# Asunatan/LM-Net

Hardware: AMD Instinct MI355X
Metric: train images/sec at 352x352, 1/2/4/8 MI355X; Dice vs ref (higher is better)
Workload: dtype f32; 1 GPU; LM-Net fp32 training step (fwd + CE/Dice loss + bwd + AdamW), batch 8/GPU, 352x352 synthetic disc masks (BASELINE configs[1]); global_batch=8, parallelism=dp1, launch=lmn_plan_run (recorded C-side schedule, one crossing per pass)

## Files before the change

### lm_net_amd/csrc/conv_wgrad.hip

```cpp
#include "conv_common.h"

namespace {

struct WgradParams {
  LmnLay lay_src[3], lay_dy;
  int32_t rpw;
  uint32_t rp_magic;
  lmn_wgrad_args_t a;
  int ntile_src[3];
  int ntile_off[3];
  int cbase[3];
  int NNTT, NMTT;
  int Cin;
  int nsets_n;
  int steps_per_img;
  int total_steps;
  float inv_keep_src[3];
  float inv_keep_dy;
  float* partial;
  int TH, TW, XH, XW, CSx, CSy, tiles_x, tiles_y, total_tiles;
  uint32_t mXW, mTW;
  int dbg;
};

__device__ __forceinline__ float* wgrad_dst(const WgradParams& P, int co, int sidx, int ch, int taps) {
  float* own = P.a.dW_src[sidx];
  return own ? own + ((int64_t)co * P.a.src[sidx].C + ch) * taps
             : P.a.dW + ((int64_t)co * P.Cin + P.cbase[sidx] + ch) * taps;
}

template <int TAPS, int NMT, int NNT, int PM = 0>
__global__ __launch_bounds__(256, 2) void wgrad_lds_kernel(const WgradParams P) {
  constexpr bool BF = PM >= 1;
  typedef typename ActT<PM>::type TA;
  const lmn_wgrad_args_t& A = P.a;
  const uint32_t soff = A.seed_ctr ? *A.seed_ctr : 0u;
  extern __shared__ __attribute__((aligned(16))) float smem[];
  const int XP = P.XH * P.XW;
  float* XS = smem;
  float* YS = smem + NNT * XP * P.CSx;
  const int tid = threadIdx.x, lane = tid & 63;
  const int wv = __builtin_amdgcn_readfirstlane(tid >> 6);
  const int q = lane >> 4, n = lane & 15;
  const int mset = blockIdx.y / P.nsets_n, nset = blockIdx.y - mset * P.nsets_n;
  const int mt0 = mset * NMT, nt0 = nset * NNT;
  const int pad = A.ksize >> 1;
  const int NP = P.TH * P.TW;

  const TA* tptr[NNT];
  const float* tscale[NNT];
  int tC[NNT], tcs[NNT], tflags[NNT], tch0[NNT];
  uint32_t tseed[NNT];
  float tp_[NNT], tik[NNT];
#pragma unroll
  for (int t = 0; t < NNT; ++t) {
    const int nt = nt0 + t;
    int sidx = 0;
    while (sidx + 1 < A.nsrc && nt >= P.ntile_off[sidx + 1]) ++sidx;
    tptr[t] = (const TA*)A.src[sidx].ptr;
    tscale[t] = A.src[sidx].scale;
    tC[t] = nt < P.NNTT ? A.src[sidx].C : 0;
    tcs[t] = A.src[sidx].cstride;
    tflags[t] = A.src[sidx].flags;
    tseed[t] = A.src[sidx].drop_seed + soff;
    tp_[t] = A.src[sidx].drop_p;
    tik[t] = P.inv_keep_src[sidx];
    tch0[t] = (nt - P.ntile_off[sidx]) * 16;
  }

  f32x4 acc[TAPS][NMT][NNT];
  float bsum[NMT];
#pragma unroll
  for (int tp = 0; tp < TAPS; ++tp)
#pragma unroll
    for (int m = 0; m < NMT; ++m)
#pragma unroll
      for (int t = 0; t < NNT; ++t) acc[tp][m][t] = f32x4{0.f, 0.f, 0.f, 0.f};
#pragma unroll
  for (int m = 0; m < NMT; ++m) bsum[m] = 0.f;

  const int t_begin = (int)(((int64_t)blockIdx.x * P.total_tiles) / gridDim.x);
  const int t_end = (int)(((int64_t)(blockIdx.x + 1) * P.total_tiles) / gridDim.x);
  for (int tile = t_begin; tile < t_end; ++tile) {
    const int b = tile / (P.tiles_x * P.tiles_y), tt = tile - b * P.tiles_x * P.tiles_y;
    const int oy0 = (tt / P.tiles_x) * P.TH, ox0 = (tt % P.tiles_x) * P.TW;
    const int iy0 = oy0 * A.stride - pad, ix0 = ox0 * A.stride - pad;
    __syncthreads();
    constexpr int UX = (TAPS == 9 && NMT * NNT == 4) ? 3 : 4, UY = 2;
    const int NXI = P.XH * P.XW * 4, NYI = NP * 4;
    for (int rd = 0; rd * (UX * 256) < NXI || rd * (UY * 256) < NYI; ++rd) {
      f32x4 vx[UX][NNT], vy[UY][NMT];
      int gpx[UX], gpy[UY];
#pragma unroll
      for (int u = 0; u < UX; ++u) {
        const int i = rd * (UX * 256) + u * 256 + tid;
        const int j = i & 3, pix = i >> 2;
        bool inb;
        int gp;
        if constexpr (TAPS == 1) {
          inb = i < NXI && ox0 + pix < A.Wout;
          gp = inb ? b * A.Wout + ox0 + pix : 0;
        } else {
          const int r = (int)__umulhi((uint32_t)pix, P.mXW), c = pix - r * P.XW;
          const int iy = iy0 + r, ix = ix0 + c;
          inb = i < NXI && (unsigned)iy < (unsigned)A.Hin && (unsigned)ix < (unsigned)A.Win;
// ... 754 lines not shown
      for (int h = 0; h < U / 4; ++h) {
        uint2 af[NMT], bf[NNT];
#pragma unroll
        for (int m = 0; m < NMT; ++m) {
          bsum[m] += (av[4 * h][m] + av[4 * h + 1][m]) + (av[4 * h + 2][m] + av[4 * h + 3][m]);
          af[m] = uint2{pk_bf16(av[4 * h][m], av[4 * h + 1][m]), pk_bf16(av[4 * h + 2][m], av[4 * h + 3][m])};
        }
#pragma unroll
        for (int t = 0; t < NNT; ++t) bf[t] = uint2{pk_bf16(bv[4 * h][t], bv[4 * h + 1][t]), pk_bf16(bv[4 * h + 2][t], bv[4 * h + 3][t])};
#pragma unroll
        for (int t = 0; t < NNT; ++t)
#pragma unroll
          for (int m = 0; m < NMT; ++m) acc[m][t] = mfma_bf16(af[m], bf[t], acc[m][t]);
      }
    } else {
#pragma unroll
    for (int u = 0; u < U; ++u) {
#pragma unroll
      for (int m = 0; m < NMT; ++m) bsum[m] += av[u][m];
#pragma unroll
      for (int t = 0; t < NNT; ++t)
#pragma unroll
        for (int m = 0; m < NMT; ++m) acc[m][t] = __builtin_amdgcn_mfma_f32_16x16x4f32(av[u][m], bv[u][t], acc[m][t], 0, 0, 0);
    }
    }
  }

  constexpr int NT = NMT * NNT;
  __shared__ float s_acc[NT * 256 + NMT * 16];
  for (int w = 0; w < 4; ++w) {
    if (wvb == w) {
#pragma unroll
      for (int m = 0; m < NMT; ++m)
#pragma unroll
        for (int t = 0; t < NNT; ++t)
#pragma unroll
          for (int r = 0; r < 4; ++r) {
            float* d = &s_acc[((m * NNT + t) * 4 + r) * 64 + lane];
            *d = (w == 0) ? acc[m][t][r] : *d + acc[m][t][r];
          }
#pragma unroll
      for (int m = 0; m < NMT; ++m) {
        float v = bsum[m];
        v += __shfl_xor(v, 16, 64);
        v += __shfl_xor(v, 32, 64);
        if (q == 0) {
          float* d = &s_acc[NT * 256 + m * 16 + n];
          *d = (w == 0) ? v : *d + v;
        }
      }
    }
    __syncthreads();
  }
  const int tid = threadIdx.x;
  if (P.partial) {
    float* dst = P.partial + ((int64_t)blockIdx.y * gridDim.x + blockIdx.x) * (NT * 256 + NMT * 16);
    for (int i = tid; i < NT * 256 + NMT * 16; i += 256) dst[i] = s_acc[i];
    return;
  }
  for (int i = tid; i < NT * 256; i += 256) {
    const int ln = i & 63, r = (i >> 6) & 3, tl = i >> 8;
    const int t = tl % NNT, m = tl / NNT;
    const int qq = ln >> 4, nn = ln & 15;
    const int co = (mt0 + m) * 16 + qq * 4 + r;
    const int nt = nt0 + t;
    if ((mt0 + m) >= P.NMTT || co >= A.Cout || nt >= P.NNTT) continue;
    int sidx = 0;
    while (sidx + 1 < A.nsrc && nt >= P.ntile_off[sidx + 1]) ++sidx;
    const int ch = (nt - P.ntile_off[sidx]) * 16 + nn;
    if (ch >= A.src[sidx].C) continue;
    atomicAdd(wgrad_dst(P, co, sidx, ch, 1), s_acc[i]);
  }
  if (A.db && nset == 0) {
    for (int i = tid; i < NMT * 16; i += 256) {
      const int co = mt0 * 16 + i;
      if (co < A.Cout && (mt0 + i / 16) < P.NMTT) {
        atomicAdd(A.db + co, s_acc[NT * 256 + i]);
        if (A.db2) atomicAdd(A.db2 + co, s_acc[NT * 256 + i]);
      }
    }
  }
}

template <int NMT, int NNT, int PM>
__global__ __launch_bounds__(256) void wgrad_1x1w_kernel(const WgradParams P) {
  constexpr int PMB = PM & 3;
  constexpr bool RP = (PM & 4) != 0;
  constexpr bool BF = PMB >= 1;
  typedef typename ActT<PMB>::type TA;
  constexpr int NTT = NMT + NNT;
  const lmn_wgrad_args_t& A = P.a;
  const uint32_t soff = A.seed_ctr ? *A.seed_ctr : 0u;
  extern __shared__ __attribute__((aligned(16))) float smem[];
  const int lane = threadIdx.x & 63;
  const int q = lane >> 4, n = lane & 15;
  const int wvb = __builtin_amdgcn_readfirstlane(threadIdx.x >> 6);
  float* WS = smem + wvb * (NTT * 256);
  const int wave = blockIdx.x * 4 + wvb, nwaves = gridDim.x * 4;
  const int mset = blockIdx.y / P.nsets_n, nset = blockIdx.y - mset * P.nsets_n;
  const int mt0 = mset * NMT, nt0 = nset * NNT;
  const int HW = A.Hout * A.Wout;
  const int NPX = A.B * HW;
  const int lp = lane >> 2, lq = lane & 3;
  constexpr int LNOFF = (4 * NTT * 256 > NMT * NNT * 256 + NMT * 16) ? 4 * NTT * 256 : NMT * NNT * 256 + NMT * 16;
  float* s_gb = smem + LNOFF;
  const bool ln = (A.src[0].flags & LMN_SRC_LN) != 0;
  if (ln) {
    for (int i = threadIdx.x; i < NNT * 16; i += 256) {
      const int t = i >> 4, c = i & 15, ch = (nt0 + t) * 16 + c;
      const bool cok = (nt0 + t) < P.NNTT && ch < A.src[0].C;
      s_gb[t * 32 + c] = cok ? A.src[0].ln_gamma[ch] : 0.f;
      s_gb[t * 32 + 16 + c] = cok ? A.src[0].ln_beta[ch] : 0.f;
    }
    __syncthreads();
  }
  float2 lnmr = float2{0.f, 1.f};

  const TA* sptr[NNT];
  const float* sscale[NNT];
  int sC[NNT], scs[NNT], sflags[NNT], sch4[NNT];
  uint32_t scho[NNT], srf[NNT];
  uint32_t sseed[NNT];
  float sp[NNT], sik[NNT];
#pragma unroll
  for (int t = 0; t < NNT; ++t) {
    const int nt = nt0 + t;
    int s = 0;
    while (s + 1 < A.nsrc && nt >= P.ntile_off[s + 1]) ++s;
    const int ch = (nt - P.ntile_off[s]) * 16 + lq * 4;
    sptr[t] = (const TA*)A.src[s].ptr;
    sscale[t] = A.src[s].scale;
    sC[t] = A.src[s].C;
    scs[t] = RP ? P.lay_src[s].cs : A.src[s].cstride;
    srf[t] = RP ? (uint32_t)P.lay_src[s].rf : 0u;
    sflags[t] = A.src[s].flags;
    sseed[t] = A.src[s].drop_seed + soff;
    sp[t] = A.src[s].drop_p;
    sik[t] = P.inv_keep_src[s];
    sch4[t] = (nt < P.NNTT && ch < A.src[s].C) ? ch : -1;
    scho[t] = (uint32_t)((sch4[t] >= 0 ? sch4[t] : 0) >> 2) * (uint32_t)P.lay_src[s].qs;
  }
  int mco4[NMT];
#pragma unroll
  for (int m = 0; m < NMT; ++m) mco4[m] = ((mt0 + m) < P.NMTT && (mt0 + m) * 16 + lq * 4 < A.Cout) ? (mt0 + m) * 16 + lq * 4 : -1;
  uint32_t mcho[NMT];
#pragma unroll
  for (int m = 0; m < NMT; ++m) mcho[m] = (uint32_t)((mco4[m] >= 0 ? mco4[m] : 0) >> 2) * (uint32_t)P.lay_dy.qs;

  f32x4 acc[NMT][NNT];
  float bsum[NMT];
#pragma unroll
  for (int m = 0; m < NMT; ++m) {
    bsum[m] = 0.f;
#pragma unroll
    for (int t = 0; t < NNT; ++t) acc[m][t] = f32x4{0.f, 0.f, 0.f, 0.f};
  }

  const int total_chunks = (NPX + 15) >> 4;
  const int cb = (int)(((int64_t)wave * total_chunks) / nwaves), ce = (int)(((int64_t)(wave + 1) * total_chunks) / nwaves);
  f32x4 stg[NTT];
  auto chunk_load = [&](int c) {
    const int px = c * 16 + lp;
    const int ps = px < NPX ? px : 0;
    if (ln) lnmr = *reinterpret_cast<const float2*>(A.src[0].ln_stats + 2 * (int64_t)ps);
    if constexpr (RP) {
      const uint32_t rowp = lmn_div_row((uint32_t)ps, (uint32_t)P.rpw, P.rp_magic);
#pragma unroll
      for (int m = 0; m < NMT; ++m) stg[m] = ld4((const TA*)A.dy + ((uint32_t)(ps * P.lay_dy.cs) + mcho[m] + rowp * (uint32_t)P.lay_dy.rf));
#pragma unroll
      for (int t = 0; t < NNT; ++t) stg[NMT + t] = ld4(sptr[t] + ((uint32_t)(ps * scs[t]) + scho[t] + rowp * srf[t]));
    } else {
#pragma unroll
      for (int m = 0; m < NMT; ++m) stg[m] = ld4((const TA*)A.dy + (uint32_t)(ps * A.dy_cstride + (mco4[m] >= 0 ? mco4[m] : 0)));
#pragma unroll
      for (int t = 0; t < NNT; ++t) stg[NMT + t] = ld4(sptr[t] + (uint32_t)(ps * scs[t] + (sch4[t] >= 0 ? sch4[t] : 0)));
    }
  };
  auto chunk_put = [&](int c) {
    const int px = c * 16 + lp;
    const bool ok = px < NPX;
    const int ps = ok ? px : 0;
#pragma unroll
    for (int m = 0; m < NMT; ++m) {
      f32x4 v = stg[m];
      if (A.dy_flags & LMN_SRC_DROP) {
#pragma unroll
        for (int k = 0; k < 4; ++k) v[k] *= lmn_drop_scale(A.dy_seed + soff, (uint32_t)(ps * A.Cout + (mco4[m] >= 0 ? mco4[m] : 0) + k), A.dy_p, P.inv_keep_dy);
      }
      if (!(ok && mco4[m] >= 0)) v = f32x4{0.f, 0.f, 0.f, 0.f};
      *reinterpret_cast<f32x4*>(&WS[m * 256 + lp * 16 + lq * 4]) = v;
    }
#pragma unroll
    for (int t = 0; t < NNT; ++t) {
      f32x4 v = stg[NMT + t];
      const int chs = sch4[t] >= 0 ? sch4[t] : 0;
      if (ln) v = (v - lnmr.x) * lnmr.y * (*reinterpret_cast<const f32x4*>(&s_gb[t * 32 + lq * 4])) + (*reinterpret_cast<const f32x4*>(&s_gb[t * 32 + 16 + lq * 4]));
      if (sflags[t] & LMN_SRC_GELU) {
#pragma unroll
        for (int k = 0; k < 4; ++k) v[k] = lmn_gelu(v[k]);
      }
      if (sflags[t] & LMN_SRC_DROP) {
#pragma unroll
        for (int k = 0; k < 4; ++k) v[k] *= lmn_drop_scale(sseed[t], (uint32_t)(ps * sC[t] + chs + k), sp[t], sik[t]);
      }
      if (sscale[t]) v *= ld4(sscale[t] + (ps / HW) * sC[t] + chs);
      if (!(ok && sch4[t] >= 0)) v = f32x4{0.f, 0.f, 0.f, 0.f};
      *reinterpret_cast<f32x4*>(&WS[(NMT + t) * 256 + lp * 16 + lq * 4]) = v;
    }
  };
  if (cb < ce) chunk_load(cb);
  for (int c = cb; c < ce; ++c) {
    chunk_put(c);
    if (c + 1 < ce) chunk_load(c + 1);
    if constexpr (BF) {
      uint2 af[NMT], bf_[NNT];
#pragma unroll
      for (int m = 0; m < NMT; ++m) {
        const float a0 = WS[m * 256 + (4 * q) * 16 + n], a1 = WS[m * 256 + (4 * q + 1) * 16 + n];
        const float a2 = WS[m * 256 + (4 * q + 2) * 16 + n], a3 = WS[m * 256 + (4 * q + 3) * 16 + n];
        bsum[m] += (a0 + a1) + (a2 + a3);
        af[m] = uint2{pk_bf16(a0, a1), pk_bf16(a2, a3)};
      }
#pragma unroll
      for (int t = 0; t < NNT; ++t) {
        const float* b = &WS[(NMT + t) * 256 + (4 * q) * 16 + n];
        bf_[t] = uint2{pk_bf16(b[0], b[16]), pk_bf16(b[32], b[48])};
      }
#pragma unroll
      for (int t = 0; t < NNT; ++t)
#pragma unroll
        for (int m = 0; m < NMT; ++m) acc[m][t] = mfma_bf16(af[m], bf_[t], acc[m][t]);
    } else {
#pragma unroll
      for (int k = 0; k < 4; ++k) {
        float av[NMT], bv[NNT];
#pragma unroll
        for (int m = 0; m < NMT; ++m) av[m] = WS[m * 256 + (4 * k + q) * 16 + n];
#pragma unroll
        for (int t = 0; t < NNT; ++t) bv[t] = WS[(NMT + t) * 256 + (4 * k + q) * 16 + n];
#pragma unroll
        for (int m = 0; m < NMT; ++m) bsum[m] += av[m];
#pragma unroll
        for (int t = 0; t < NNT; ++t)
#pragma unroll
          for (int m = 0; m < NMT; ++m) acc[m][t] = __builtin_amdgcn_mfma_f32_16x16x4f32(av[m], bv[t], acc[m][t], 0, 0, 0);
      }
    }
  }

  constexpr int NT = NMT * NNT;
  __syncthreads();
  float* s_acc = smem;
  for (int w = 0; w < 4; ++w) {
    if (wvb == w) {
#pragma unroll
      for (int m = 0; m < NMT; ++m)
#pragma unroll
        for (int t = 0; t < NNT; ++t)
#pragma unroll
          for (int r = 0; r < 4; ++r) {
            float* d = &s_acc[((m * NNT + t) * 4 + r) * 64 + lane];
            *d = (w == 0) ? acc[m][t][r] : *d + acc[m][t][r];
          }
#pragma unroll
      for (int m = 0; m < NMT; ++m) {
        float v = bsum[m];
        v += __shfl_xor(v, 16, 64);
        v += __shfl_xor(v, 32, 64);
        if (q == 0) {
          float* d = &s_acc[NT * 256 + m * 16 + n];
          *d = (w == 0) ? v : *d + v;
        }
      }
    }
    __syncthreads();
  }
  const int tid = threadIdx.x;
  if (P.partial) {
    float* dst = P.partial + ((int64_t)blockIdx.y * gridDim.x + blockIdx.x) * (NT * 256 + NMT * 16);
    for (int i = tid; i < NT * 256 + NMT * 16; i += 256) dst[i] = s_acc[i];
    return;
  }
  for (int i = tid; i < NT * 256; i += 256) {
    const int ln = i & 63, r = (i >> 6) & 3, tl = i >> 8;
    const int t = tl % NNT, m = tl / NNT;
    const int qq = ln >> 4, nn = ln & 15;
    const int co = (mt0 + m) * 16 + qq * 4 + r;
    const int nt = nt0 + t;
    if ((mt0 + m) >= P.NMTT || co >= A.Cout || nt >= P.NNTT) continue;
    int sidx = 0;
    while (sidx + 1 < A.nsrc && nt >= P.ntile_off[sidx + 1]) ++sidx;
    const int ch = (nt - P.ntile_off[sidx]) * 16 + nn;
    if (ch >= A.src[sidx].C) continue;
    atomicAdd(wgrad_dst(P, co, sidx, ch, 1), s_acc[i]);
  }
  if (A.db && nset == 0) {
    for (int i = tid; i < NMT * 16; i += 256) {
      const int co = mt0 * 16 + i;
      if (co < A.Cout && (mt0 + i / 16) < P.NMTT) {
        atomicAdd(A.db + co, s_acc[NT * 256 + i]);
        if (A.db2) atomicAdd(A.db2 + co, s_acc[NT * 256 + i]);
      }
    }
  }
}

template <int TAPS, int NMT, int NNT>
__global__ __launch_bounds__(1024) void wgrad_reduce_kernel(const WgradParams P, int nblk, int ksl) {
  const lmn_wgrad_args_t& A = P.a;
  constexpr int NT = TAPS * NMT * NNT, PER = NT * 256 + NMT * 16;
  __shared__ __attribute__((aligned(16))) float red[4096];
  const int mset = blockIdx.y / P.nsets_n, nset = blockIdx.y - mset * P.nsets_n;
  const int mt0 = mset * NMT, nt0 = nset * NNT;
  const float* src = P.partial + (int64_t)blockIdx.y * nblk * PER;
  const int epq = 1024 / ksl, epb = epq * 4;
  const int q = threadIdx.x & (epq - 1), ks = threadIdx.x / epq;
  const int i4 = (blockIdx.x * epq + q) * 4;
  f32x4 s4 = f32x4{0.f, 0.f, 0.f, 0.f};
  if (i4 < PER) {
    const float* sp = src + i4;
#pragma unroll 4
    for (int k = ks; k < nblk; k += ksl) s4 += *reinterpret_cast<const f32x4*>(sp + (int64_t)k * PER);
  }
  *reinterpret_cast<f32x4*>(&red[threadIdx.x * 4]) = s4;
  __syncthreads();
  for (int e = threadIdx.x; e < epb; e += 1024) {
  const int i = blockIdx.x * epb + e;
  if (i >= PER) return;
  float sum = 0.f;
  for (int k = 0; k < ksl; ++k) sum += red[k * epb + e];
  if (i < NT * 256) {
// ... 162 lines not shown
};

static int wgrad_setup(const lmn_wgrad_args_t& A, WgradParams& P, WgGeom& G) {
  LMN_REQUIRE(A.ksize == 1 || A.ksize == 3, "conv_wgrad: ksize %d", A.ksize);
  LMN_REQUIRE(A.stride == 1 || A.stride == 2, "conv_wgrad: stride %d", A.stride);
  LMN_REQUIRE(A.nsrc >= 1 && A.nsrc <= 3, "conv_wgrad: nsrc %d", A.nsrc);
  LMN_REQUIRE(A.dy && A.Cout > 0 && A.dy_cstride >= A.Cout, "conv_wgrad: dy/Cout");
  for (int s = 0; s < A.nsrc && s < 3; ++s) LMN_REQUIRE(A.dW || A.dW_src[s], "conv_wgrad: no gradient tensor for source %d", s);
  LMN_REQUIRE(!A.db2 || A.db, "conv_wgrad: db2 without db");
  LMN_REQUIRE(A.B > 0 && A.Hout > 0 && A.Wout > 0, "conv_wgrad: empty tensor");
  LMN_REQUIRE(A.mma_dtype == LMN_F32 || A.mma_dtype == LMN_BF16, "conv_wgrad: mma_dtype %d", A.mma_dtype);
  LMN_REQUIRE(A.act_dtype == LMN_F32 || (A.act_dtype == LMN_BF16 && A.mma_dtype == LMN_BF16),
              "conv_wgrad: act_dtype %d with mma_dtype %d", A.act_dtype, A.mma_dtype);
  P.a = A;
  P.NNTT = 0;
  P.Cin = 0;
  for (int s = 0; s < 3; ++s) {
    P.ntile_src[s] = P.ntile_off[s] = P.cbase[s] = 0;
    P.inv_keep_src[s] = 1.f;
  }
  for (int s = 0; s < A.nsrc; ++s) {
    LMN_REQUIRE(A.src[s].ptr && A.src[s].C > 0 && A.src[s].cstride >= A.src[s].C, "conv_wgrad: source %d", s);
    P.ntile_src[s] = (A.src[s].C + 15) / 16;
    P.ntile_off[s] = P.NNTT;
    P.cbase[s] = P.Cin;
    P.NNTT += P.ntile_src[s];
    P.Cin += A.src[s].C;
    if (A.src[s].flags & LMN_SRC_DROP) P.inv_keep_src[s] = 1.f / (1.f - A.src[s].drop_p);
  }
  P.inv_keep_dy = (A.dy_flags & LMN_SRC_DROP) ? 1.f / (1.f - A.dy_p) : 1.f;
  {
    int rw = 0;
    for (int s = 0; s < 3; ++s) {
      const int w = s < A.nsrc ? A.src[s].rp_w : 0;
      P.lay_src[s] = lmn_lay_make(w, s < A.nsrc ? A.src[s].C : 4, s < A.nsrc ? A.src[s].cstride : 4);
      if (w) {
        LMN_REQUIRE(w > 0 && A.src[s].cstride == A.src[s].C && (rw == 0 || rw == w), "conv_wgrad: row-planar source %d must be a whole tensor (cstride == C) of the call's width", s);
        rw = w;
      }
    }
    P.lay_dy = lmn_lay_make(A.dy_rp_w, A.Cout, A.dy_cstride);
    if (A.dy_rp_w) { LMN_REQUIRE(A.dy_rp_w > 0 && A.dy_cstride == A.Cout && (rw == 0 || rw == A.dy_rp_w), "conv_wgrad: row-planar dy must be a whole tensor of the call's width"); rw = A.dy_rp_w; }
    if (rw) LMN_REQUIRE(A.ksize == 1 && A.stride == 1 && rw == A.Wout && rw == A.Win, "conv_wgrad: row-planar operands belong to 1x1 stride-1 calls over images of their own width (rp_w %d, call %d)", rw, A.Wout);
    P.rpw = rw;
    P.rp_magic = lmn_div_magic(rw);
  }
  P.NMTT = (A.Cout + 15) / 16;
  P.steps_per_img = (A.Hout * A.Wout + 3) / 4;
  LMN_REQUIRE((int64_t)A.B * P.steps_per_img < (1LL << 31), "conv_wgrad: too many pixels");
  for (int s = 0; s < A.nsrc; ++s)
    LMN_REQUIRE((int64_t)A.B * A.Hin * A.Win * A.src[s].cstride < (1LL << 31), "conv_wgrad: source %d larger than 2^31 elements", s);
  LMN_REQUIRE((int64_t)A.B * A.Hout * A.Wout * A.dy_cstride < (1LL << 31), "conv_wgrad: dy larger than 2^31 elements");
  P.total_steps = A.B * P.steps_per_img;
  if (A.ksize == 1 && A.stride == 1) {
    P.a.Wout = A.Hout * A.Wout; P.a.Hout = 1;
    P.a.Win = A.Hin * A.Win; P.a.Hin = 1;
  }
  int NMT, NNT;
  wgrad_tile_shape(A, P.NMTT, P.NNTT, &NMT, &NNT);
  const int msets = (P.NMTT + NMT - 1) / NMT;
  P.nsets_n = (P.NNTT + NNT - 1) / NNT;
  const int gy = msets * P.nsets_n;
  const int taps = A.ksize * A.ksize;
  const int64_t per = (int64_t)taps * NMT * NNT * 256 + NMT * 16;
  const lmn_wgrad_args_t& Gm = P.a;
  const bool v1c = wgrad_v1(A) && Gm.Wout >= 32 && (NMT * NNT == 4 || NMT * NNT == 1);
  const int npmax = Gm.stride == 2 ? 64 : ((Gm.ksize == 1 || NMT * NNT == 1 || (Gm.Wout <= 32 && !v1c)) ? 256 : 128);
  P.TW = Gm.Wout < (Gm.ksize == 1 ? npmax : 32) ? Gm.Wout : (Gm.ksize == 1 ? npmax : 32);
  if (Gm.stride == 2 && P.TW > 16) P.TW = 16;
  P.TH = npmax / P.TW;
  if (P.TH > Gm.Hout) P.TH = Gm.Hout;
  if (P.TH < 1) P.TH = 1;
  P.XH = (P.TH - 1) * Gm.stride + Gm.ksize;
  P.XW = (P.TW - 1) * Gm.stride + Gm.ksize;
  P.CSy = 16;
  P.CSx = A.stride == 1 ? 16 : 24;
  const bool bf = A.mma_dtype == LMN_BF16;
  const int pm = bf ? (A.act_dtype == LMN_BF16 ? 2 : 1) : 0;
  if (bf) P.CSy = P.CSx = 12;
  P.tiles_x = (Gm.Wout + P.TW - 1) / P.TW;
  P.tiles_y = (Gm.Hout + P.TH - 1) / P.TH;
  P.total_tiles = A.B * P.tiles_x * P.tiles_y;
  P.dbg = 0;
  LMN_REQUIRE(P.XH * P.XW < 65536 && P.TH * P.TW < 65536, "conv_wgrad: tile too large");
  P.mXW = (uint32_t)((1ull << 32) / (uint32_t)P.XW + 1);
  P.mTW = (uint32_t)((1ull << 32) / (uint32_t)P.TW + 1);
  int64_t lds_floats = (int64_t)NNT * P.XH * P.XW * P.CSx + (int64_t)NMT * P.TH * P.TW * P.CSy;
  if (lds_floats < per) lds_floats = per;
  LMN_REQUIRE(lds_floats * 4 <= 160 * 1024, "conv_wgrad: LDS tile too large (%lld B)", (long long)lds_floats * 4);
  int64_t blocks64 = P.total_tiles;
  const int64_t esz = A.act_dtype == LMN_BF16 ? 2 : 4;
  bool v1 = v1c && P.TW == 32 && P.XW == 34 &&
            P.XH * P.XW * 4 <= (NMT * NNT == 1 ? 6 : 4) * 256 && P.TH * P.TW * 4 <= (NMT * NNT == 1 ? 4 : 2) * 256 &&
            (int64_t)A.B * A.Hout * A.Wout * A.dy_cstride * esz < 0xfffffff0LL;
  for (int s = 0; s < A.nsrc; ++s) v1 = v1 && (int64_t)A.B * A.Hin * A.Win * A.src[s].cstride * esz < 0xfffffff0LL;
  bool up2 = false;
  for (int s = 0; s < A.nsrc; ++s) up2 = up2 || (A.src[s].flags & LMN_SRC_UP2) != 0;
  if (v1) {
    const int ux = NMT * NNT == 1 ? 6 : 4, uy = NMT * NNT == 1 ? 4 : 2, cs = bf ? 12 : 16;
    lds_floats = (int64_t)(NNT * ux + NMT * uy) * 64 * cs;
    if (up2) lds_floats += (int64_t)NNT * (NMT * NNT == 1 ? 3 : 2) * 64 * 16;
    if (NMT * NNT == 1 && lds_floats < per) lds_floats = per;
  }
  if (up2) {
    LMN_REQUIRE(A.nsrc == 1 && A.ksize == 3 && A.stride == 1 && A.Hin % 2 == 0 && A.Win % 2 == 0 && !(A.src[0].flags & ~LMN_SRC_UP2) && !A.src[0].scale,
                "conv_wgrad: LMN_SRC_UP2 belongs to single-source 3x3 stride-1 calls (Hin x Win = the upsampled size) without other source transforms");
    LMN_REQUIRE(v1 && (P.XH + 1) / 2 + 2 <= (NMT * NNT == 1 ? 3 : 2) * 64 / 19,
                "conv_wgrad: LMN_SRC_UP2 needs the wgrad3 form (upsampled map >= 32 wide; lmn_conv_wgrad_up2_ok says so beforehand)");
  }
  static int cap_other = -1;
  if (cap_other < 0) { const char* e = getenv("LMN_WGRAD_CAP_OTHER"); cap_other = e && atoi(e) > 0 ? atoi(e) : 512; }
  const int btot = v1 ? wgrad_blocks_total(A) : cap_other;
  const int64_t cap = btot / gy > 2 ? btot / gy : 2;
  if (blocks64 > cap) blocks64 = cap;
  if (blocks64 < 1) blocks64 = 1;
  bool rp_any = A.dy_rp_w != 0, ln_any = false;
  for (int s = 0; s < A.nsrc; ++s) { rp_any = rp_any || A.src[s].rp_w != 0; ln_any = ln_any || (A.src[s].flags & LMN_SRC_LN) != 0; }
  G.direct = A.ksize == 1 && A.stride == 1 && ((int64_t)Gm.Hout * Gm.Wout >= 32 || rp_any || ln_any);
  if (G.direct) {
    const int64_t steps = ((int64_t)A.B * Gm.Hout * Gm.Wout + 3) / 4;
    blocks64 = (steps + 63) / 64;
    if (blocks64 > cap) blocks64 = cap;
    if (blocks64 < 1) blocks64 = 1;
  }
  P.partial = nullptr;
  if (A.workspace && (wgrad_two_stage(gy, blocks64, per) || (g_lmn_det && blocks64 > 1)) && (int64_t)gy * blocks64 * per <= A.workspace_floats) {
    P.partial = A.workspace;
  } else if (g_lmn_det) {
    blocks64 = 1;
  } else if (blocks64 > 512 / gy && 512 / gy >= 2) {
    blocks64 = 512 / gy;
  }
  G.NMT = NMT; G.NNT = NNT; G.gy = gy; G.taps = taps; G.per = per; G.blocks = (int)blocks64;
  G.v1 = v1; G.pm = pm; G.shmem = (size_t)lds_floats * 4;
  bool any_tf = (A.dy_flags & LMN_SRC_DROP) != 0;
  for (int s = 0; s < A.nsrc; ++s) any_tf = any_tf || A.src[s].flags != 0 || A.src[s].scale != nullptr;
  const bool old_shape = (NMT == 1 && NNT <= 4) || (NNT == 1 && NMT <= 4) || (NMT == 2 && NNT == 2);
  G.wave_staged = !(pm == 2 && !any_tf && old_shape) || (rp_any && (int64_t)Gm.Hout * Gm.Wout < 32);
  for (int s = 0; s < A.nsrc; ++s) {
    if (A.src[s].flags & LMN_SRC_LN) {
      LMN_REQUIRE(A.nsrc == 1 && G.direct && G.wave_staged && !rp_any, "conv_wgrad: LMN_SRC_LN belongs to single-source NHWC 1x1 stride-1 calls");
      LMN_REQUIRE(A.src[s].ln_gamma && A.src[s].ln_beta && A.src[s].ln_stats, "conv_wgrad: LMN_SRC_LN needs ln_gamma / ln_beta and the ln_stats table of the forward conv");
      LMN_REQUIRE(!(A.src[s].flags & ~LMN_SRC_LN) && !A.src[s].scale, "conv_wgrad: LMN_SRC_LN does not combine with other source transforms");
    }
  }
  return 0;
}

int lmn_sizeof_reduce_job(void) { return (int)sizeof(lmn_reduce_job_t); }

int lmn_conv_wgrad_up2_ok(const lmn_wgrad_args_t* args) {
  if (!args || args->nsrc != 1 || args->ksize != 3 || args->stride != 1 || (args->Hin & 1) || (args->Win & 1)) return 0;
  if ((args->src[0].flags & ~LMN_SRC_UP2) || args->src[0].scale) return 0;
  lmn_wgrad_args_t a = *args;
  a.src[0].flags = 0;
  WgradParams P;
  WgGeom G;
  char keep[sizeof(g_lmn_err)];
  memcpy(keep, g_lmn_err, sizeof(keep));
  const int rc = wgrad_setup(a, P, G);
  memcpy(g_lmn_err, keep, sizeof(keep));
  if (rc != 0 || !G.v1) return 0;
  return (P.XH + 1) / 2 + 2 <= (G.NMT * G.NNT == 1 ? 3 : 2) * 64 / 19 ? 1 : 0;
}

int lmn_conv_wgrad_job(const lmn_wgrad_args_t* args, lmn_reduce_job_t* out) {
  LMN_REQUIRE(args && out, "conv_wgrad_job: null pointer");
  WgradParams P;
  WgGeom G;
  const int rc = wgrad_setup(*args, P, G);
  if (rc) return rc;
  memset(out, 0, sizeof(*out));
  if (!P.partial) return 0;
  const lmn_wgrad_args_t& A = *args;
  out->partial = P.partial;
  out->nblk = G.blocks; out->per = (int32_t)G.per; out->gy = G.gy; out->nsets_n = P.nsets_n;
  out->taps = G.taps; out->NMT = G.NMT; out->NNT = G.NNT; out->nsrc = A.nsrc;
  out->Cout = A.Cout; out->Cin = P.Cin; out->NMTT = P.NMTT; out->NNTT = P.NNTT;
  for (int s = 0; s < 3; ++s) {
    out->srcC[s] = s < A.nsrc ? A.src[s].C : 0;
    out->ntile_off[s] = P.ntile_off[s];
    out->cbase[s] = P.cbase[s];
    out->dW_src[s] = A.dW_src[s];
  }
  out->dW = A.dW; out->db = A.db; out->db2 = A.db2;
  out->ksl = reduce_slices(G.blocks);
  out->blocks_per_set = (int32_t)((G.per + 4096 / out->ksl - 1) / (4096 / out->ksl));
  return 0;
}
int lmn_wgrad_reduce_batch(const lmn_reduce_job_t* jobs_dev, int njobs, int64_t total_blocks, lmn_stream_t stream) {
  LMN_REC(lmn_wgrad_reduce_batch(jobs_dev, njobs, total_blocks, stream));
  LMN_REQUIRE(jobs_dev && njobs > 0 && total_blocks > 0 && total_blocks < (1LL << 31), "wgrad_reduce_batch: bad job table");
  LMN_LAUNCH(wgrad_reduce_batch_kernel, dim3((unsigned)total_blocks), dim3(1024), 0, (hipStream_t)stream, jobs_dev, njobs);
  return lmn_launch_status("wgrad_reduce_batch");
}

int lmn_conv_wgrad(const lmn_wgrad_args_t* args, lmn_stream_t stream) {
  if (args && g_lmn_rec) {
    const lmn_wgrad_args_t copy = *args;
    lmn_rec_push([copy, stream]() -> int { return lmn_conv_wgrad(&copy, stream); }, "lmn_conv_wgrad(");
  }
  LMN_REQUIRE(args, "conv_wgrad: null args");
  const lmn_wgrad_args_t& A = *args;
  WgradParams P;
  WgGeom G;
  {
    const int rc = wgrad_setup(A, P, G);
    if (rc) return rc;
  }
  if (g_lmn_prof_on) {
    const double opix = (double)A.B * A.Hout * A.Wout, ipix = (double)A.B * A.Hin * A.Win;
    lmn_prof_cost(2.0 * opix * (double)P.Cin * A.Cout * A.ksize * A.ksize, (A.act_dtype == LMN_BF16 ? 2.0 : 4.0) * (ipix * P.Cin + opix * A.Cout));
  }
  const int NMT = G.NMT, NNT = G.NNT, gy = G.gy, pm = G.pm, blocks = G.blocks;
  const int64_t per = G.per;
  const bool v1 = G.v1;
  const bool reduce_now = P.partial && !A.defer_reduce;
  const size_t shmem = G.shmem;
  hipStream_t st = (hipStream_t)stream;
  const dim3 grid(blocks, gy);
#define LMN_WG(T, M, N)                                                                                             \
  do {                                                                                                              \
    if (shmem > 64 * 1024) {                                                                                        \
      (void)hipFuncSetAttribute((const void*)wgrad_lds_kernel<T, M, N, 0>, hipFuncAttributeMaxDynamicSharedMemorySize, (int)shmem); \
      (void)hipFuncSetAttribute((const void*)wgrad_lds_kernel<T, M, N, 1>, hipFuncAttributeMaxDynamicSharedMemorySize, (int)shmem); \
      (void)hipFuncSetAttribute((const void*)wgrad_lds_kernel<T, M, N, 2>, hipFuncAttributeMaxDynamicSharedMemorySize, (int)shmem); \
    }                                                                                                               \
    if constexpr (T == 9 && (M * N == 4 || M * N == 1)) {                                                           \
      if (v1) {                                                                                                     \
        if (pm == 2) wgrad3_launch<M, N, 2>(grid, shmem, st, P);                                                    \
        else if (pm == 1) wgrad3_launch<M, N, 1>(grid, shmem, st, P);                                               \
        else wgrad3_launch<M, N, 0>(grid, shmem, st, P);                                                            \
        goto wg_reduce_##T##M##N;                                                                                   \
      }                                                                                                             \
    }                                                                                                               \
    if (pm == 2) LMN_LAUNCH((wgrad_lds_kernel<T, M, N, 2>), grid, dim3(256), shmem, st, P);                 \
    else if (pm == 1) LMN_LAUNCH((wgrad_lds_kernel<T, M, N, 1>), grid, dim3(256), shmem, st, P);            \
    else LMN_LAUNCH((wgrad_lds_kernel<T, M, N, 0>), grid, dim3(256), shmem, st, P);                         \
  wg_reduce_##T##M##N:                                                                                              \
    if (reduce_now) {                                                                                               \
      const int ksl = reduce_slices(blocks);                                                                        \
      const int rb = (int)((per + 4096 / ksl - 1) / (4096 / ksl));                                                    \
      LMN_LAUNCH((wgrad_reduce_kernel<T, M, N>), dim3(rb, gy), dim3(1024), 0, st, P, blocks, ksl);          \
    }                                                                                                               \
  } while (0)
  if (G.direct) {
    const int64_t nb = blocks;
    const dim3 dgrid((unsigned)nb, gy);
    const bool wave_staged = G.wave_staged;
#define LMN_WDK(KERN, M, N, SH)                                                                                    \
  do {                                                                                                              \
    if (P.rpw) {                                 \
      if (pm == 2) LMN_LAUNCH((KERN<M, N, 6>), dgrid, dim3(256), SH, st, P);                                        \
      else if (pm == 1) LMN_LAUNCH((KERN<M, N, 5>), dgrid, dim3(256), SH, st, P);                                   \
      else LMN_LAUNCH((KERN<M, N, 4>), dgrid, dim3(256), SH, st, P);                                                \
    } else if (pm == 2) LMN_LAUNCH((KERN<M, N, 2>), dgrid, dim3(256), SH, st, P);                                   \
    else if (pm == 1) LMN_LAUNCH((KERN<M, N, 1>), dgrid, dim3(256), SH, st, P);                                     \
    else LMN_LAUNCH((KERN<M, N, 0>), dgrid, dim3(256), SH, st, P);                                                  \
  } while (0)
#define LMN_WD(M, N)                                                                                               \
  do {                                                                                                              \
    if (wave_staged) {                                                                                              \
      const int64_t stf = 4 * (M + N) * 256, rdf = (int64_t)M * N * 256 + M * 16;                                   \
      const size_t wsh = (size_t)((stf > rdf ? stf : rdf) + 32 * N) * 4;    \
      LMN_WDK(wgrad_1x1w_kernel, M, N, wsh);                                                                        \
    } else LMN_WDK(wgrad_1x1_kernel, M, N, 0);                                                                      \
    if (reduce_now) {                                                                                               \
      const int ksl = reduce_slices((int)nb);                                                                       \
      const int rb = (int)((per + 4096 / ksl - 1) / (4096 / ksl));                                                    \
      LMN_LAUNCH((wgrad_reduce_kernel<1, M, N>), dim3(rb, gy), dim3(1024), 0, st, P, (int)nb, ksl);         \
    }                                                                                                               \
  } while (0)
#define LMN_WW(M, N)                                                                                               \
  do {                                                                                                              \
    const int64_t stf = 4 * (M + N) * 256, rdf = (int64_t)M * N * 256 + M * 16;                                     \
    const size_t wsh = (size_t)((stf > rdf ? stf : rdf) + 32 * N) * 4;                                              \
    LMN_WDK(wgrad_1x1w_kernel, M, N, wsh);                                                                          \
    if (reduce_now) {                                                                                               \
      const int ksl = reduce_slices((int)nb);                                                                       \
      const int rb = (int)((per + 4096 / ksl - 1) / (4096 / ksl));                                                    \
      LMN_LAUNCH((wgrad_reduce_kernel<1, M, N>), dim3(rb, gy), dim3(1024), 0, st, P, (int)nb, ksl);         \
    }                                                                                                               \
  } while (0)
    switch (NMT * 8 + NNT) {
      case 1 * 8 + 1: LMN_WD(1, 1); break;
      case 1 * 8 + 2: LMN_WD(1, 2); break;
      case 1 * 8 + 3: LMN_WD(1, 3); break;
      case 1 * 8 + 4: LMN_WD(1, 4); break;
      case 2 * 8 + 1: LMN_WD(2, 1); break;
      case 3 * 8 + 1: LMN_WD(3, 1); break;
      case 4 * 8 + 1: LMN_WD(4, 1); break;
      case 2 * 8 + 2: LMN_WD(2, 2); break;
      case 2 * 8 + 3: LMN_WW(2, 3); break;
      case 3 * 8 + 2: LMN_WW(3, 2); break;
      case 2 * 8 + 4: LMN_WW(2, 4); break;
      default: LMN_WW(4, 2); break;
    }
#undef LMN_WW
#undef LMN_WD
#undef LMN_WDK
    return lmn_launch_status("conv_wgrad(1x1)");
  }
#define LMN_WGS(T)                                                   \
  do {                                                               \
    if (NMT == 1 && NNT == 1) LMN_WG(T, 1, 1);                       \
    else if (NMT == 1) LMN_WG(T, 1, 2);                              \
    else if (NNT == 1) LMN_WG(T, 2, 1);                              \
    else LMN_WG(T, 2, 2);                                            \
  } while (0)
  if (A.ksize == 1) LMN_WGS(1); else LMN_WGS(9);
#undef LMN_WGS
#undef LMN_WG
  return lmn_launch_status("conv_wgrad");
}

}
```

Baseline: 589.3 images/sec.

## Stream 1x1 wgrad operands into an LDS ring via buffer_load-to-LDS

For the non-bf16 path, the wave-staged 1x1 weight-gradient kernel now loads dy and source tiles directly from global memory into a per-wave LDS ring using buffer_load ... lds, with vmcnt waits, instead of staging through registers. Elementwise transforms (dropout, GELU, scale) are then applied in place in LDS. The next chunk's load is issued once the current chunk's LDS reads are done. Ring depth comes from an env var and defaults to 1, and the kernel also gains a waves_per_eu occupancy hint. The aim is to overlap global loads with MFMA work and free registers, at the cost of inline assembly, extra LDS and extra read-modify-write passes over LDS.

```diff
diff --git a/lm_net_amd/csrc/conv_wgrad.hip b/lm_net_amd/csrc/conv_wgrad.hip
--- a/lm_net_amd/csrc/conv_wgrad.hip
+++ b/lm_net_amd/csrc/conv_wgrad.hip
@@ -21,6 +21,7 @@
   int TH, TW, XH, XW, CSx, CSy, tiles_x, tiles_y, total_tiles;
   uint32_t mXW, mTW;
   int dbg;
+  int ring;
 };
 
 __device__ __forceinline__ float* wgrad_dst(const WgradParams& P, int co, int sidx, int ch, int taps) {
@@ -941,8 +942,27 @@
   }
 }
 
+typedef int wg_i32x4 __attribute__((ext_vector_type(4)));
+constexpr unsigned WG_OOB = 0x80000000u;
+__device__ __forceinline__ wg_i32x4 wg_rsrc(const void* p) {
+  const unsigned long long a = (unsigned long long)p;
+  wg_i32x4 r;
+  r.x = __builtin_amdgcn_readfirstlane((int)(unsigned)a);
+  r.y = __builtin_amdgcn_readfirstlane((int)(unsigned)(a >> 32));
+  r.z = (int)WG_OOB;
+  r.w = 0x00020000;
+  return r;
+}
+__device__ __forceinline__ void wg_piece(unsigned ldsaddr, unsigned voff, wg_i32x4 rsrc) {
+  unsigned keep;
+  asm volatile("s_mov_b32 %0, m0\n\ts_mov_b32 m0, %1\n\ts_nop 0\n\tbuffer_load_dwordx4 %2, %3, 0 offen lds\n\ts_mov_b32 m0, %0"
+               : "=&s"(keep) : "s"(ldsaddr), "v"(voff), "s"(rsrc) : "memory");
+}
+template <int N> __device__ __forceinline__ void wg_wait() { asm volatile("s_waitcnt vmcnt(%0)" ::"n"(N) : "memory"); }
+
 template <int NMT, int NNT, int PM>
-__global__ __launch_bounds__(256) void wgrad_1x1w_kernel(const WgradParams P) {
+__global__ __launch_bounds__(256) __attribute__((amdgpu_waves_per_eu(NNT == 1 && NMT <= 2 ? 8 : 1)))
+void wgrad_1x1w_kernel(const WgradParams P) {
   constexpr int PMB = PM & 3;
   constexpr bool RP = (PM & 4) != 0;
   constexpr bool BF = PMB >= 1;
@@ -1035,17 +1055,32 @@
       for (int t = 0; t < NNT; ++t) stg[NMT + t] = ld4(sptr[t] + (uint32_t)(ps * scs[t] + (sch4[t] >= 0 ? sch4[t] : 0)));
     }
   };
+  auto dy_tf = [&](f32x4 v, int m, int ps) {
+    if (A.dy_flags & LMN_SRC_DROP) {
+#pragma unroll
+      for (int k = 0; k < 4; ++k) v[k] *= lmn_drop_scale(A.dy_seed + soff, (uint32_t)(ps * A.Cout + (mco4[m] >= 0 ? mco4[m] : 0) + k), A.dy_p, P.inv_keep_dy);
+    }
+    return v;
+  };
+  auto src_tf = [&](f32x4 v, int t, int ps) {
+    const int chs = sch4[t] >= 0 ? sch4[t] : 0;
+    if (sflags[t] & LMN_SRC_GELU) {
+#pragma unroll
+      for (int k = 0; k < 4; ++k) v[k] = lmn_gelu(v[k]);
+    }
+    if (sflags[t] & LMN_SRC_DROP) {
+#pragma unroll
+      for (int k = 0; k < 4; ++k) v[k] *= lmn_drop_scale(sseed[t], (uint32_t)(ps * sC[t] + chs + k), sp[t], sik[t]);
+    }
+    return v;
+  };
   auto chunk_put = [&](int c) {
     const int px = c * 16 + lp;
     const bool ok = px < NPX;
     const int ps = ok ? px : 0;
 #pragma unroll
     for (int m = 0; m < NMT; ++m) {
-      f32x4 v = stg[m];
-      if (A.dy_flags & LMN_SRC_DROP) {
-#pragma unroll
-        for (int k = 0; k < 4; ++k) v[k] *= lmn_drop_scale(A.dy_seed + soff, (uint32_t)(ps * A.Cout + (mco4[m] >= 0 ? mco4[m] : 0) + k), A.dy_p, P.inv_keep_dy);
-      }
+      f32x4 v = dy_tf(stg[m], m, ps);
       if (!(ok && mco4[m] >= 0)) v = f32x4{0.f, 0.f, 0.f, 0.f};
       *reinterpret_cast<f32x4*>(&WS[m * 256 + lp * 16 + lq * 4]) = v;
     }
@@ -1054,23 +1089,13 @@
       f32x4 v = stg[NMT + t];
       const int chs = sch4[t] >= 0 ? sch4[t] : 0;
       if (ln) v = (v - lnmr.x) * lnmr.y * (*reinterpret_cast<const f32x4*>(&s_gb[t * 32 + lq * 4])) + (*reinterpret_cast<const f32x4*>(&s_gb[t * 32 + 16 + lq * 4]));
-      if (sflags[t] & LMN_SRC_GELU) {
-#pragma unroll
-        for (int k = 0; k < 4; ++k) v[k] = lmn_gelu(v[k]);
-      }
-      if (sflags[t] & LMN_SRC_DROP) {
-#pragma unroll
-        for (int k = 0; k < 4; ++k) v[k] *= lmn_drop_scale(sseed[t], (uint32_t)(ps * sC[t] + chs + k), sp[t], sik[t]);
-      }
+      v = src_tf(v, t, ps);
       if (sscale[t]) v *= ld4(sscale[t] + (ps / HW) * sC[t] + chs);
       if (!(ok && sch4[t] >= 0)) v = f32x4{0.f, 0.f, 0.f, 0.f};
       *reinterpret_cast<f32x4*>(&WS[(NMT + t) * 256 + lp * 16 + lq * 4]) = v;
     }
   };
-  if (cb < ce) chunk_load(cb);
-  for (int c = cb; c < ce; ++c) {
-    chunk_put(c);
-    if (c + 1 < ce) chunk_load(c + 1);
+  auto chunk_mma = [&](const float* WS, auto&& reads_done) __attribute__((always_inline)) {
     if constexpr (BF) {
       uint2 af[NMT], bf_[NNT];
 #pragma unroll
@@ -1085,27 +1110,112 @@
         const float* b = &WS[(NMT + t) * 256 + (4 * q) * 16 + n];
         bf_[t] = uint2{pk_bf16(b[0], b[16]), pk_bf16(b[32], b[48])};
       }
+      reads_done();
 #pragma unroll
       for (int t = 0; t < NNT; ++t)
 #pragma unroll
         for (int m = 0; m < NMT; ++m) acc[m][t] = mfma_bf16(af[m], bf_[t], acc[m][t]);
     } else {
+      float av[4][NMT], bv[4][NNT];
 #pragma unroll
       for (int k = 0; k < 4; ++k) {
-        float av[NMT], bv[NNT];
-#pragma unroll
-        for (int m = 0; m < NMT; ++m) av[m] = WS[m * 256 + (4 * k + q) * 16 + n];
-#pragma unroll
-        for (int t = 0; t < NNT; ++t) bv[t] = WS[(NMT + t) * 256 + (4 * k + q) * 16 + n];
-#pragma unroll
-        for (int m = 0; m < NMT; ++m) bsum[m] += av[m];
+#pragma unroll
+        for (int m = 0; m < NMT; ++m) av[k][m] = WS[m * 256 + (4 * k + q) * 16 + n];
+#pragma unroll
+        for (int t = 0; t < NNT; ++t) bv[k][t] = WS[(NMT + t) * 256 + (4 * k + q) * 16 + n];
+      }
+      reads_done();
+#pragma unroll
+      for (int k = 0; k < 4; ++k) {
+#pragma unroll
+        for (int m = 0; m < NMT; ++m) bsum[m] += av[k][m];
 #pragma unroll
         for (int t = 0; t < NNT; ++t)
 #pragma unroll
-          for (int m = 0; m < NMT; ++m) acc[m][t] = __builtin_amdgcn_mfma_f32_16x16x4f32(av[m], bv[t], acc[m][t], 0, 0, 0);
-      }
-    }
-  }
+          for (int m = 0; m < NMT; ++m) acc[m][t] = __builtin_amdgcn_mfma_f32_16x16x4f32(av[k][m], bv[k][t], acc[m][t], 0, 0, 0);
+      }
+    }
+  };
+  if constexpr (PMB != 2) {
+    const int D = P.ring > 1 ? P.ring : 1, nch = ce - cb;
+    float* const WR = smem + wvb * (D * NTT * 256);
+    const unsigned ring0 = (unsigned)(size_t)(__attribute__((address_space(3))) void*)smem + (unsigned)(wvb * D * NTT) * 1024u;
+    auto chunk_issue = [&](int i, int slot) __attribute__((always_inline)) {
+      const int px = (cb + i) * 16 + lp;
+      const bool ok = px < NPX;
+      const int ps = ok ? px : 0;
+      const unsigned s0 = ring0 + (unsigned)(slot * NTT) * 1024u;
+      uint32_t rowp = 0;
+      if constexpr (RP) rowp = lmn_div_row((uint32_t)ps, (uint32_t)P.rpw, P.rp_magic);
+#pragma unroll
+      for (int m = 0; m < NMT; ++m) {
+        const uint32_t e = RP ? (uint32_t)(ps * P.lay_dy.cs) + mcho[m] + rowp * (uint32_t)P.lay_dy.rf : (uint32_t)(ps * A.dy_cstride + (mco4[m] >= 0 ? mco4[m] : 0));
+        const uint32_t e0 = __builtin_amdgcn_readfirstlane(e);
+        wg_piece(__builtin_amdgcn_readfirstlane(s0 + (unsigned)m * 1024u), (ok && mco4[m] >= 0) ? (e - e0) * 4u : WG_OOB, wg_rsrc((const float*)A.dy + e0));
+      }
+#pragma unroll
+      for (int t = 0; t < NNT; ++t) {
+        const uint32_t e = RP ? (uint32_t)(ps * scs[t]) + scho[t] + rowp * srf[t] : (uint32_t)(ps * scs[t] + (sch4[t] >= 0 ? sch4[t] : 0));
+        const uint32_t e0 = __builtin_amdgcn_readfirstlane(e);
+        wg_piece(__builtin_amdgcn_readfirstlane(s0 + (unsigned)(NMT + t) * 1024u), (ok && sch4[t] >= 0) ? (e - e0) * 4u : WG_OOB, wg_rsrc((const float*)sptr[t] + e0));
+      }
+    };
+    for (int i = 0; i < D && i < nch; ++i) chunk_issue(i, i);
+    int slot = 0;
+    for (int i = 0; i < nch; ++i) {
+      const int px = (cb + i) * 16 + lp;
+      const bool ok = px < NPX;
+      const int ps = ok ? px : 0;
+      f32x4 scv[NNT];
+#pragma unroll
+      for (int t = 0; t < NNT; ++t)
+        if (sscale[t]) scv[t] = ld4(sscale[t] + (ps / HW) * sC[t] + (sch4[t] >= 0 ? sch4[t] : 0));
+      if (ln) lnmr = *reinterpret_cast<const float2*>(A.src[0].ln_stats + 2 * (int64_t)ps);
+      const int after = nch - i - 1 < D - 1 ? nch - i - 1 : D - 1;
+      if (after == 0) wg_wait<0>();
+      else if (after == 1) wg_wait<NTT>();
+      else if (after == 2) wg_wait<2 * NTT>();
+      else wg_wait<3 * NTT>();
+      float* const S = WR + slot * (NTT * 256);
+      if (A.dy_flags & LMN_SRC_DROP) {
+#pragma unroll
+        for (int m = 0; m < NMT; ++m) {
+          f32x4* const d = reinterpret_cast<f32x4*>(&S[m * 256 + lp * 16 + lq * 4]);
+          f32x4 v = dy_tf(*d, m, ps);
+          if (!(ok && mco4[m] >= 0)) v = f32x4{0.f, 0.f, 0.f, 0.f};
+          *d = v;
+        }
+      }
+#pragma unroll
+      for (int t = 0; t < NNT; ++t) {
+        if (sflags[t] || sscale[t]) {
+          f32x4* const d = reinterpret_cast<f32x4*>(&S[(NMT + t) * 256 + lp * 16 + lq * 4]);
+          f32x4 v = *d;
+          if (ln) v = (v - lnmr.x) * lnmr.y * (*reinterpret_cast<const f32x4*>(&s_gb[t * 32 + lq * 4])) + (*reinterpret_cast<const f32x4*>(&s_gb[t * 32 + 16 + lq * 4]));
+          v = src_tf(v, t, ps);
+          if (sscale[t]) v *= scv[t];
+          if (!(ok && sch4[t] >= 0)) v = f32x4{0.f, 0.f, 0.f, 0.f};
+          *d = v;
+        }
+      }
+      asm volatile("" ::: "memory");
+      chunk_mma(S, [&]() __attribute__((always_inline)) {
+        if (i + D < nch) {
+          asm volatile("s_waitcnt lgkmcnt(0)" ::: "memory");
+          chunk_issue(i + D, slot);
+        }
+      });
+      slot = slot + 1 == D ? 0 : slot + 1;
+    }
+  } else {
+    if (cb < ce) chunk_load(cb);
+    for (int c = cb; c < ce; ++c) {
+      chunk_put(c);
+      if (c + 1 < ce) chunk_load(c + 1);
+      chunk_mma(WS, []() {});
+    }
+  }
+
 
   constexpr int NT = NMT * NNT;
   __syncthreads();
@@ -1434,6 +1544,7 @@
   P.tiles_y = (Gm.Hout + P.TH - 1) / P.TH;
   P.total_tiles = A.B * P.tiles_x * P.tiles_y;
   P.dbg = 0;
+  P.ring = 0;
   LMN_REQUIRE(P.XH * P.XW < 65536 && P.TH * P.TW < 65536, "conv_wgrad: tile too large");
   P.mXW = (uint32_t)((1ull << 32) / (uint32_t)P.XW + 1);
   P.mTW = (uint32_t)((1ull << 32) / (uint32_t)P.TW + 1);
@@ -1497,6 +1608,18 @@
     }
   }
   return 0;
+}
+
+static int wgrad_ring_depth(const lmn_wgrad_args_t& A, const WgGeom& G) {
+  if (!(G.direct && G.wave_staged) || G.pm == 2) return 1;
+  for (int s = 0; s < A.nsrc; ++s)
+    if (A.src[s].flags & LMN_SRC_LN) return 1;
+  const int ntt = G.NMT + G.NNT;
+  int d = 1;
+  const char* e = getenv("LMN_WGRAD_RING");
+  if (e && atoi(e) >= 1) d = atoi(e) < 4 ? atoi(e) : 4;
+  if (d > 16 / ntt) d = 16 / ntt;
+  return d >= 1 ? d : 1;
 }
 
 int lmn_sizeof_reduce_job(void) { return (int)sizeof(lmn_reduce_job_t); }
@@ -1600,6 +1723,8 @@
     const int64_t nb = blocks;
     const dim3 dgrid((unsigned)nb, gy);
     const bool wave_staged = G.wave_staged;
+    P.ring = wgrad_ring_depth(A, G);
+    const int slots = P.ring;
 #define LMN_WDK(KERN, M, N, SH)                                                                                    \
   do {                                                                                                              \
     if (P.rpw) {                                 \
@@ -1613,7 +1738,7 @@
 #define LMN_WD(M, N)                                                                                               \
   do {                                                                                                              \
     if (wave_staged) {                                                                                              \
-      const int64_t stf = 4 * (M + N) * 256, rdf = (int64_t)M * N * 256 + M * 16;                                   \
+      const int64_t stf = 4 * slots * (M + N) * 256, rdf = (int64_t)M * N * 256 + M * 16;                           \
       const size_t wsh = (size_t)((stf > rdf ? stf : rdf) + 32 * N) * 4;    \
       LMN_WDK(wgrad_1x1w_kernel, M, N, wsh);                                                                        \
     } else LMN_WDK(wgrad_1x1_kernel, M, N, 0);                                                                      \
@@ -1625,7 +1750,7 @@
   } while (0)
 #define LMN_WW(M, N)                                                                                               \
   do {                                                                                                              \
-    const int64_t stf = 4 * (M + N) * 256, rdf = (int64_t)M * N * 256 + M * 16;                                     \
+    const int64_t stf = 4 * slots * (M + N) * 256, rdf = (int64_t)M * N * 256 + M * 16;                             \
     const size_t wsh = (size_t)((stf > rdf ? stf : rdf) + 32 * N) * 4;                                              \
     LMN_WDK(wgrad_1x1w_kernel, M, N, wsh);                                                                          \
     if (reduce_now) {                                                                                               \
```

After: 587.3 images/sec. About the same (-0.3%).
